# Naxaes/Rust-Swift-Raytracer

Measured on AMD Instinct MI355X. Metric: Mrays/sec + frames/sec at 1920×1080 spp=64; 1/2/4/8 MI355X, higher is better.
Workload: dtype f32; 1 GPU; c2: 1920x1080, spp 64, depth 8, 486 spheres, 0 triangles, COUNTER RNG; width=1920, height=1080, spp=64, depth=8, parallelism=one device renders the frame in place (no RCCL call)

## Files before the change

### rust-swift-raytracer_amd/csrc/render.h

```cpp
#pragma once

#include <hip/hip_runtime.h>

#include <cstdint>

#include "fastdiv.h"

namespace rtamd {

enum : uint32_t { kRngCounter = 1, kRngReplay = 2 };
enum : uint32_t { kRngSerialCount = 3, kRngSerialEstimate = 4, kRngSerialCheck = 5, kRngSerialCoalesce = 6,
                  kRngSerialPixel = 7 };
enum : uint32_t { kMatDiffuse = 0, kMatMetal = 1, kMatDielectric = 2, kMatEmission = 3 };
constexpr uint32_t kPrimaryTriStripW = 8;
#ifndef RT_TRACE_RING
#define RT_TRACE_RING 4
#endif
constexpr uint32_t kTraceRing = RT_TRACE_RING;
#ifdef RT_STAMPS
constexpr uint32_t kStatSlots = 24;
#else
constexpr uint32_t kStatSlots = 16;
#endif
constexpr uint32_t kStampSegs = 8;
// ... 16 lines not shown
    const float4 *tri_hot;
    const float4 *tri_geo;
    const float *mats;
    float *samples;
    float *ring;
    uint32_t ring_shift;
    uint32_t *out;
    float inv_spp;
    uint32_t alpha_u8;
    uint32_t *job_counter;
    uint32_t *job_counter_next;
    unsigned long long *stats;
    const uint32_t *replay;
    float cam[12];
    float wden, hden;
    float wrcp, hrcp;
    uint32_t xdiv_uv;
    uint32_t nsph, nsph_padded, ntri;
    uint32_t width, height, spp;
    int32_t depth;
    uint32_t mode, seed;
    uint32_t row_block, rank, nranks;
    uint32_t slab_row0;
    uint32_t njobs;
    uint32_t npix;
    uint32_t chunk;
    uint32_t nparts;
    const float4 *bvh_nodes;
    const uint32_t *bvh_miss;
    const uint16_t *bvh_miss16;
    const float4 *bvh_prims;
    const uint32_t *bvh_prim_id;
    const float4 *big_hot;
    const uint32_t *big_id;
    uint32_t nnodes, nbig, nprims;
    uint32_t use_lds;
    uint32_t ablate;
    const float4 *sph_shade;
    const uint32_t *sph_kind;
    FastDiv div_spp, div_width, div_rowblock;
    uint32_t refill_min;
    uint32_t walk_min;
    uint32_t tri_walk_min;
    uint32_t steps;
    uint32_t step;
    float bvh_c[3], bvh_r, bvh_rmax, bvh_mag, bvh_inv_rmin;
    const uint4 *tbvh_nodes;
    const float4 *tbvh_tris;
    const uint32_t *tbvh_loose;
    uint32_t tnodes, ttris, tloose;
    float tbvh_c[3], tbvh_r, tbvh_mag;
    float tbvh_oc[3];
    float tq_base[3], tq_step[3], tq_nbase, tq_nstep;
    const uint4 *tw_nodes;
    uint32_t tw_depth;
    uint32_t wsteps;
    float cq_base[3], cq_step[3];
    const uint4 *cam_nodes;
    const float4 *cam_tris;
    uint32_t cam_nnodes;
    const uint32_t *ptl_off;
    const uint32_t *ptl_items;
    uint32_t ptl_spr;
    uint32_t ptl_always, ptl_end;
    const uint2 *spl;
    const uint32_t *win;
    SerialPred sM;
    const uint32_t *slo;
    const uint32_t *ctrl;
    uint32_t cbase;
    uint32_t nserial;
    uint32_t sspp;
    FastDiv div_sspp;
    uint32_t max_draws;
    uint32_t sL, sK;
    uint32_t gj32, gj_c0, gj_2p;
    const float4 *tw_tris;
    uint32_t tw_stride, tc_ncells;
    uint32_t tc_n[3];
    float tc_lo[3], tc_size, tc_inv_size;
    const uint4 *spix;
};

RT_HOST_DEVICE inline uint32_t serial_lo(const SerialPred &M, uint32_t a, uint32_t jl, uint32_t K,
                                         uint32_t depth, uint32_t nserial) {
    const uint32_t j = a + jl < nserial ? a + jl : nserial;
    double c = __builtin_floor(serial_M(M, j) - serial_M(M, a)) - (double)(K / 2u);
    const double hi = (double)depth * (double)jl;
    c = c < 0.0 ? 0.0 : c;
    c = c > hi ? hi : c;
    return (uint32_t)c;
}

hipError_t launch_trace(const TraceParams &p, uint32_t blocks, hipStream_t stream,
                        const uint4 *corner = nullptr);
hipError_t launch_sphere_lists(const float4 *prims, uint32_t n, const double *Mi, const double *o,
                               double e_abs, double wden, double hden, uint32_t width, uint32_t height,
                               int4 *rects, uint32_t *flag, uint2 *rec, hipStream_t stream);
size_t serial_tab_doubles(uint32_t npix);
hipError_t launch_serial_check_count(const float *flags, uint32_t n, unsigned long long *count,
                                     hipStream_t stream);
hipError_t launch_serial_moments(const float *est, uint32_t pix0, uint32_t n, uint32_t spp, uint32_t R,
                                 double scale, double *tab, uint32_t npix, hipStream_t stream);
hipError_t launch_serial_tables(double *tab, double *scratch, uint32_t npix, uint32_t spp, uint32_t L,
                                uint32_t n0, hipStream_t stream);
size_t serial_scan_scratch(uint32_t npix);
constexpr uint32_t kSerialWinPerThread = 4;
constexpr uint32_t kSerialJumpT1 = 4096 / kSerialWinPerThread;
constexpr uint32_t kSerialJumpWords = 32 * (64 + kSerialJumpT1 + 256);
hipError_t launch_serial_window(uint32_t *ctrl, const uint32_t *jump, uint32_t *win, uint32_t n,
                                SerialPred M, uint32_t *lo, uint32_t L, uint32_t K, uint32_t depth,
                                uint32_t nserial, uint32_t pix_spp, uint32_t pix_emax, uint32_t *counters,
                                uint32_t ncounters, uint4 *spix, uint32_t pix_chunk, const uint4 *spix_prev,
                                hipStream_t stream);
hipError_t launch_serial_reuse(const uint32_t *ctrl, const uint4 *spix, const uint4 *spix_prev, float *ptab,
                               const float *ptab_prev, uint32_t npq_max, uint32_t spp, uint32_t L,
                               uint32_t nserial, hipStream_t stream);
hipError_t launch_serial_pixtab_gather(const uint32_t *ctrl, const float *ptab, const uint32_t *lo, float *table,
                                       uint32_t L, uint32_t K, uint32_t spp, uint32_t nserial, hipStream_t stream);
inline uint64_t serial_pixtab_emax64(uint64_t spp, uint64_t K, uint64_t depth) {
    return 2u * (spp - 1u) + 3u * (depth * (spp - 1u) + K) + 1u;
}
hipError_t launch_serial_coalesce(const TraceParams &p, uint32_t *path, uint32_t *bend, uint32_t L, uint32_t Kmax,
                                  uint32_t R, bool tree_lds, unsigned long long *dbg, hipStream_t stream);
size_t serial_coalesce_lds(const TraceParams &p, uint32_t K, bool tree_lds);
size_t serial_coalesce_search_lds(uint32_t K, uint32_t depth);
uint32_t serial_walk_block(uint32_t L);
constexpr uint32_t kMaxWalkBlocks = 4096;
constexpr uint32_t kWalkFinWords = 4 + kMaxWalkBlocks;
constexpr uint32_t kMaxWalkR = 256;
constexpr uint32_t kWalkLdsRowBytes = 48 * 1024;
constexpr uint32_t kWalkLdsMaxPix = 72;
hipError_t launch_serial_walk(uint32_t *ctrl, const float *table, SerialPred M, const double *V,
                              uint32_t npix, uint32_t spp, float z, float sfloor, const uint32_t *win,
                              uint32_t *states, uint32_t *bend, uint32_t *path, uint32_t *fin,
                              const uint32_t *lo, uint32_t *sbend, uint32_t *sB, uint32_t L, uint32_t Lw,
                              uint32_t K, uint32_t R, uint32_t depth, uint32_t nserial, const float *ptab,
                              uint32_t lds_rows, hipStream_t stream);
uint32_t serial_super_words(uint32_t L, uint32_t K, uint32_t R);
hipError_t launch_resolve_ex(const float *samples, uint32_t *out, uint32_t npix, uint32_t spp,
                             float inv_spp, uint32_t width, uint32_t slab_row0,
                             hipStream_t stream);
hipError_t launch_assemble(const uint32_t *gathered, uint32_t *out, uint32_t width, uint32_t height,
                           uint32_t row_block, uint32_t nranks, uint32_t max_rows,
                           hipStream_t stream);
hipError_t trace_occupancy(int *blocks_per_cu, int variant, size_t lds_bytes, bool step, int mesh,
                           int kind);
inline int trace_mesh_kind(bool triangles, bool tree) { return !triangles ? 0 : tree ? 2 : 1; }
size_t trace_lds_bytes(const TraceParams &p, bool corner = false);
__host__ __device__ inline size_t trace_tree_lds(uint32_t nnodes, uint32_t nprims, uint32_t nsph_padded) {
    return (size_t)nnodes * 64 + (size_t)nprims * 20 + (size_t)nsph_padded * 36;
}
__host__ __device__ inline size_t trace_corner_lds(uint32_t nnodes, uint32_t nprims) {
    return (size_t)nnodes * 128 + (size_t)nprims * 20;
}
constexpr size_t kLdsPerCu = 160 * 1024, kLdsDefaultMax = 64 * 1024;
hipError_t trace_lds_opt_in();
constexpr uint32_t kLdsTreeMaxNodes = 1023;
uint32_t trace_block_threads(bool lds, int mesh, int kind);
size_t trace_dyn_lds(const TraceParams &p, bool lds, bool wide, uint32_t threads, bool corner = false);

}
```

### rust-swift-raytracer_amd/csrc/render.hip

```cpp
#include <hip/hip_runtime.h>

#include <cstdint>
#include <type_traits>

#include "exactdiv.h"
#include "render.h"

#pragma clang fp contract(off)

namespace rtamd {
namespace {

struct F3 { float x, y, z; };

__device__ __forceinline__ F3 f3(float x, float y, float z) { return F3{x, y, z}; }
__device__ __forceinline__ F3 operator+(F3 a, F3 b) { return F3{a.x + b.x, a.y + b.y, a.z + b.z}; }
__device__ __forceinline__ F3 operator-(F3 a, F3 b) { return F3{a.x - b.x, a.y - b.y, a.z - b.z}; }
__device__ __forceinline__ F3 operator-(F3 a) { return F3{-a.x, -a.y, -a.z}; }
__device__ __forceinline__ F3 scale(F3 a, float s) { return F3{a.x * s, a.y * s, a.z * s}; }
__device__ __forceinline__ float dot(F3 a, F3 b) { return (a.x * b.x + a.y * b.y) + a.z * b.z; }
__device__ __forceinline__ F3 cross(F3 a, F3 b) {
    return F3{a.y * b.z - a.z * b.y, -(a.x * b.z - a.z * b.x), a.x * b.y - a.y * b.x};
}
__device__ __forceinline__ F3 divide_by(F3 a, float b) {
// ... 148 lines not shown
    const float r2 = -hb + sq;
    const bool v1 = tmin < r1;
    const float c = v1 ? r1 : r2;
    const bool valid = v1 || (tmin < r2);
    const uint64_t kc = ((uint64_t)__float_as_uint(c) << 32) | (uint32_t)idx;
    const uint64_t kb = ((uint64_t)__float_as_uint(best_t) << 32) | (uint32_t)best_i;
    const bool take = valid && c != __builtin_inff() && kc < kb;
    if (take) { best_t = c; best_i = idx; }
    return take;
}

constexpr float kErrK = 3.0e-3f;

struct BvhView {
    const float4 *nodes;
    const uint32_t *miss32;
    const uint16_t *miss16;
    const float4 *prims;
    const uint32_t *ids;
    const float4 *shade;
    const uint32_t *kinds;
};

__device__ __forceinline__ float slab_rcp(float d) {
    return __builtin_amdgcn_fmed3f(__builtin_amdgcn_rcpf(d), -1e20f, 1e20f);
}

struct SphBound { float A, e_abs; };
__device__ __forceinline__ SphBound sph_bound(const TraceParams &p, F3 org) {
    const float ax = org.x - p.bvh_c[0], ay = org.y - p.bvh_c[1], az = org.z - p.bvh_c[2];
    return SphBound{__builtin_amdgcn_sqrtf((ax * ax + ay * ay) + az * az) * 1.00001f + p.bvh_r,
                    2e-6f * ((fabsf(org.x) + fabsf(org.y)) + fabsf(org.z) + p.bvh_mag)};
}
constexpr float kErrKq = 40.5f * 0x1p-24f;
__device__ __forceinline__ float sph_inflation(const TraceParams &p, SphBound b, float bt) {
    const float s = fminf(b.A, bt + p.bvh_rmax) * (1.0f + 3.0f * kErrK) + p.bvh_rmax;
    return fminf(kErrK * s, (kErrKq * s) * (s * p.bvh_inv_rmin)) + b.e_abs;
}

__device__ __forceinline__ void spheres_big(const TraceParams &p, F3 org, F3 dir, float &best_t,
                                            int &best_i) {
    for (uint32_t k = 0; k < p.nbig; ++k) {
        const float4 S = uniform_load(p.big_hot, k);
        sphere_candidate(S, org, dir, (int)uniform_load_u32(p.big_id, k), best_t, best_i);
    }
}

template <bool kLds>
__device__ __forceinline__ bool sphere_node(const BvhView &v, F3 inv, uint32_t ooff, float best_t, F3 nlo,
                                            F3 nhi, uint32_t &node, uint32_t &leaf, uint32_t &node_tests) {
    ++node_tests;
    float4 B0, B1;
    uint32_t miss, hit = 0;
    if (kLds) {
#if defined(__HIP_DEVICE_COMPILE__)
        typedef const __attribute__((address_space(3))) char *lds_cptr;
        const lds_cptr rec = (lds_cptr)(uintptr_t)node;
        B0 = *(const __attribute__((address_space(3))) float4 *)rec;
        B1 = *(const __attribute__((address_space(3))) float4 *)(rec + 16);
        const uint32_t lw = *(const __attribute__((address_space(3))) uint32_t *)(rec + 32 + ooff);
        hit = lw & 0xFFFFu;
        miss = lw >> 16;
#else
        B0 = B1 = make_float4(0.0f, 0.0f, 0.0f, 0.0f);
        miss = 0;
#endif
    } else {
        B0 = v.nodes[2 * node];
        B1 = v.nodes[2 * node + 1];
        miss = v.miss32[8 * node + ooff];
    }
    const float t0x = __builtin_fmaf(B0.x, inv.x, nlo.x), t1x = __builtin_fmaf(B1.x, inv.x, nhi.x);
    const float t0y = __builtin_fmaf(B0.y, inv.y, nlo.y), t1y = __builtin_fmaf(B1.y, inv.y, nhi.y);
    const float t0z = __builtin_fmaf(B0.z, inv.z, nlo.z), t1z = __builtin_fmaf(B1.z, inv.z, nhi.z);
    const float tn = fmaxf(fmaxf(fminf(t0x, t1x), fminf(t0y, t1y)), fminf(t0z, t1z));
    const float tf = fminf(fminf(fmaxf(t0x, t1x), fmaxf(t0y, t1y)), fmaxf(t0z, t1z));
    const bool skip = tn > tf || tf < 0.001f || __float_as_int(tn) > __float_as_int(best_t);
    if (kLds) {
        leaf = __float_as_uint(B0.w);
        node = skip ? miss : hit;
        return !skip && leaf != 0u;
    }
    const uint32_t a = __float_as_uint(B0.w);
    const bool is_leaf = (a & kLeafBitDev) != 0;
    const uint32_t child = a + ((ooff >> __float_as_uint(B1.w)) & 1u);
    node = (skip || is_leaf) ? miss : child;
    leaf = ((a & ~kLeafBitDev) << 3) | __float_as_uint(B1.w);
    return !skip && is_leaf;
}

__device__ __forceinline__ bool sphere_node_corner(uint32_t offn, uint32_t offf, F3 inv, float best_t, F3 nn,
                                                   F3 nf, uint32_t &node, uint32_t &leaf, uint32_t &node_tests) {
    ++node_tests;
#if defined(__HIP_DEVICE_COMPILE__)
    typedef float f3v __attribute__((ext_vector_type(3)));
    uint32_t an, af;
    asm("v_lshl_add_u32 %0, %1, 7, %2" : "=v"(an) : "v"(node), "v"(offn));
    asm("v_lshl_add_u32 %0, %1, 7, %2" : "=v"(af) : "v"(node), "v"(offf));
    const float4 N = *(const __attribute__((address_space(3))) float4 *)(uintptr_t)an;
    const f3v Fc = *(const __attribute__((address_space(3))) f3v *)(uintptr_t)af;
    const float tnx = __builtin_fmaf(N.x, inv.x, nn.x), tfx = __builtin_fmaf(Fc.x, inv.x, nf.x);
    const float tny = __builtin_fmaf(N.y, inv.y, nn.y), tfy = __builtin_fmaf(Fc.y, inv.y, nf.y);
    const float tnz = __builtin_fmaf(N.z, inv.z, nn.z), tfz = __builtin_fmaf(Fc.z, inv.z, nf.z);
    const float tn = fmaxf(fmaxf(tnx, tny), tnz);
    const float tf = fminf(fminf(tfx, tfy), tfz);
    const bool skip = tn > tf || tf < 0.001f || __float_as_int(tn) > __float_as_int(best_t);
    const uint32_t lw = __float_as_uint(N.w);
    const bool is_leaf = (int32_t)lw < 0;
    node = (skip || is_leaf) ? (lw & 0xFFFFu) : (lw >> 16);
    leaf = (lw >> 16) & 0x7FFFu;
    return !skip && is_leaf;
#else
    (void)offn; (void)offf; (void)inv; (void)best_t; (void)nn; (void)nf;
    node = 0xFFFFu;
    leaf = 0;
    return false;
#endif
}

__device__ __forceinline__ uint32_t sphere_corner_entry(uint32_t lbase, uint32_t oct, uint32_t nnodes) {
#if defined(__HIP_DEVICE_COMPILE__)
    if (nnodes > 1u)
        return *(const __attribute__((address_space(3))) uint32_t *)(uintptr_t)(lbase + 16u * oct + 12u) >> 16;
#endif
    (void)lbase; (void)oct; (void)nnodes;
    return 0;
}

__device__ __forceinline__ void sphere_corner_slabs(F3 org, F3 inv, float e, uint32_t oct, F3 &nn, F3 &nf) {
    const float ex = (oct & 1u) ? -e : e, ey = (oct & 2u) ? -e : e, ez = (oct & 4u) ? -e : e;
    nn = f3(-((org.x + ex) * inv.x), -((org.y + ey) * inv.y), -((org.z + ez) * inv.z));
    nf = f3(-((org.x - ex) * inv.x), -((org.y - ey) * inv.y), -((org.z - ez) * inv.z));
}

template <bool kLds>
__device__ __forceinline__ uint32_t sphere_walk_entry(uint32_t root, uint32_t oct, uint32_t nnodes) {
#if defined(__HIP_DEVICE_COMPILE__)
    if (kLds && nnodes > 1u) {
        typedef const __attribute__((address_space(3))) char *lds_cptr;
        return *(const __attribute__((address_space(3))) uint32_t *)((lds_cptr)(uintptr_t)root + 32 + 4u * oct) &
               0xFFFFu;
    }
#endif
    (void)oct;
    (void)nnodes;
    return root;
}

__device__ __forceinline__ void sphere_slabs(F3 org, F3 inv, float e, F3 &nlo, F3 &nhi) {
    nlo = f3(-((org.x + e) * inv.x), -((org.y + e) * inv.y), -((org.z + e) * inv.z));
    nhi = f3(-((org.x - e) * inv.x), -((org.y - e) * inv.y), -((org.z - e) * inv.z));
}

__device__ __forceinline__ void sphere_leaf(const BvhView &v, F3 org, F3 dir, uint32_t leaf, float &best_t,
                                            int &best_i, uint32_t &sph_tests) {
    const uint32_t first = leaf >> 3, n = leaf & 7u;
#ifndef RT_LEAF_LOOP
    sph_tests += n;
    sphere_candidate(v.prims[first], org, dir, (int)v.ids[first], best_t, best_i);
    if (n > 1u) {
        sphere_candidate(v.prims[first + 1], org, dir, (int)v.ids[first + 1], best_t, best_i);
        for (uint32_t j = first + 2; j < first + n; ++j)
            sphere_candidate(v.prims[j], org, dir, (int)v.ids[j], best_t, best_i);
    }
#else
    for (uint32_t j = first; j < first + n; ++j) {
        ++sph_tests;
        sphere_candidate(v.prims[j], org, dir, (int)v.ids[j], best_t, best_i);
    }
#endif
}

__device__ __forceinline__ bool tri_edges(F3 n, F3 v0, F3 v1, F3 v2, F3 pt) {
    if (dot(n, cross(v1 - v0, pt - v0)) < 0.0f) return false;
    if (dot(n, cross(v2 - v1, pt - v1)) < 0.0f) return false;
    if (dot(n, cross(v0 - v2, pt - v2)) < 0.0f) return false;
    return true;
}

__device__ __forceinline__ bool tri_plane(float4 N, F3 org, F3 dir, float best_t, float &t) {
    const float cosl = (N.x * dir.x + N.y * dir.y) + N.z * dir.z;
    if (-1e-8f < cosl && cosl < 1e-8f) return false;
    t = (((N.x * org.x + N.y * org.y) + N.z * org.z) + N.w) / cosl;
    return !(t < 0.001f || t > best_t);
}

__device__ __forceinline__ void triangles_brute(const TraceParams &p, F3 org, F3 dir, float best_t,
                                                float &tri_t, int &tri_i, uint32_t &tri_in) {
    const float tmin = 0.001f;
    for (uint32_t j = 0; j < p.ntri; ++j) {
        const float4 N = p.tri_hot[j];
        const float cosl = (N.x * dir.x + N.y * dir.y) + N.z * dir.z;
        if (-1e-8f < cosl && cosl < 1e-8f) continue;
        const float t = (((N.x * org.x + N.y * org.y) + N.z * org.z) + N.w) / cosl;
        if (t < tmin || t > best_t) continue;
        ++tri_in;
        const float4 *g = p.tri_geo + 4u * j;
        const float4 A = g[0], B = g[1], Cc = g[2];
        if (!tri_edges(f3(N.x, N.y, N.z), f3(A.x, A.y, A.z), f3(B.x, B.y, B.z), f3(Cc.x, Cc.y, Cc.z),
                       org + scale(dir, t)))
            continue;
        if (t < tri_t) { tri_t = t; tri_i = (int)j; }
    }
}

__device__ __forceinline__ bool tri_merge(float t, int idx, float &tri_t, int &tri_i) {
    const bool take = t < tri_t || (t == tri_t && tri_t < __builtin_inff() && idx < tri_i);
    if (take) { tri_t = t; tri_i = idx; }
    return take;
}

__device__ __forceinline__ bool tri_record(const float4 *r, F3 org, F3 dir, float best_t,
                                           float &tri_t, int &tri_i, uint32_t &tri_in) {
    const float4 N = r[0];
    float t;
    if (!tri_plane(N, org, dir, best_t, t)) return false;
    ++tri_in;
    const float4 A = r[1], B = r[2], Cc = r[3];
    if (!tri_edges(f3(N.x, N.y, N.z), f3(A.x, A.y, A.z), f3(B.x, B.y, B.z), f3(Cc.x, Cc.y, Cc.z),
                   org + scale(dir, t)))
        return false;
    return tri_merge(t, (int)__float_as_uint(A.w), tri_t, tri_i);
}

__device__ __forceinline__ bool tri_begin(const TraceParams &p, F3 org, F3 dir, float best_t,
                                          bool cam, float &rho, float &tri_t, int &tri_i,
                                          uint32_t &tri_in, uint32_t &tri_done) {
    tri_done += p.tloose;
    for (uint32_t k = 0; k < p.tloose; ++k) {
        const uint32_t j = p.tbvh_loose[k];
        const float4 N = p.tri_hot[j];
        float t;
        if (!tri_plane(N, org, dir, best_t, t)) continue;
        ++tri_in;
        const float4 *g = p.tri_geo + 4u * j;
        const float4 A = g[0], B = g[1], Cc = g[2];
        if (tri_edges(f3(N.x, N.y, N.z), f3(A.x, A.y, A.z), f3(B.x, B.y, B.z), f3(Cc.x, Cc.y, Cc.z),
                      org + scale(dir, t)))
            tri_merge(t, (int)j, tri_t, tri_i);
    }
    const float onorm = (fabsf(org.x) + fabsf(org.y)) + fabsf(org.z);
    if (!cam && !(onorm < 1e18f)) {
        tri_done += p.ttris;
        for (uint32_t j = 0; j < p.ttris; ++j)
            tri_record(p.tbvh_tris + 4u * j, org, dir, best_t, tri_t, tri_i, tri_in);
        return false;
    }
    const float dist = ((fabsf(org.x - p.tbvh_c[0]) + fabsf(org.y - p.tbvh_c[1])) +
                        fabsf(org.z - p.tbvh_c[2])) + p.tbvh_r + 2.0f * onorm;
    rho = cam ? 0.0f : 1e-5f * ((dist + onorm) + p.tbvh_mag);
    return true;
}

__device__ __forceinline__ bool tri_node(const TraceParams &p, F3 nlo, F3 nhi, F3 inv, F3 dlt2, bool cam,
                                         float cap, uint32_t &node, uint32_t &leaf,
                                         uint32_t &node_tests) {
    ++node_tests;
    const uint4 *qn = (cam ? p.cam_nodes : p.tbvh_nodes) + 2u * node;
    const uint4 q0 = qn[0], q1 = qn[1];
    const uint32_t a = cam ? q0.w : q1.z;
    const uint32_t miss = cam ? q1.x : q1.w;
    const float gbx = cam ? p.cq_base[0] : p.tq_base[0], gsx = cam ? p.cq_step[0] : p.tq_step[0];
    const float gby = cam ? p.cq_base[1] : p.tq_base[1], gsy = cam ? p.cq_step[1] : p.tq_step[1];
    const float gbz = cam ? p.cq_base[2] : p.tq_base[2], gsz = cam ? p.cq_step[2] : p.tq_step[2];
    auto lo16 = [](uint32_t w) { return (float)(w & 0xFFFFu); };
    auto hi16 = [](uint32_t w) { return (float)(w >> 16); };
    const float4 B0 = make_float4(__builtin_fmaf(lo16(q0.x), gsx, gbx), __builtin_fmaf(hi16(q0.x), gsy, gby),
                                  __builtin_fmaf(lo16(q0.y), gsz, gbz), 0.0f);
    const float4 B1 = make_float4(__builtin_fmaf(hi16(q0.y), gsx, gbx), __builtin_fmaf(lo16(q0.z), gsy, gby),
                                  __builtin_fmaf(hi16(q0.z), gsz, gbz), 0.0f);
    const float nb = cam ? 0.0f : p.tq_nbase, ns = cam ? 0.0f : p.tq_nstep;
    const float4 N0 = make_float4(__builtin_fmaf(lo16(q0.w), ns, nb), __builtin_fmaf(hi16(q0.w), ns, nb),
                                  __builtin_fmaf(lo16(q1.x), ns, nb), 0.0f);
    const float4 N1 = make_float4(__builtin_fmaf(hi16(q1.x), ns, nb), __builtin_fmaf(lo16(q1.y), ns, nb),
                                  __builtin_fmaf(hi16(q1.y), ns, nb), 0.0f);
    const float ax = N0.x * dlt2.x, bx = N1.x * dlt2.x;
    const float ay = N0.y * dlt2.y, by = N1.y * dlt2.y;
    const float az = N0.z * dlt2.z, bz = N1.z * dlt2.z;
    const float sl = (fminf(ax, bx) + fminf(ay, by)) + fminf(az, bz);
    const float sh = (fmaxf(ax, bx) + fmaxf(ay, by)) + fmaxf(az, bz);
    auto widen = [&](float lo, float hi, float m0, float m1, float nl, float nh, float iv, float &t0,
                     float &t1) {
        const float a = sl * m0, b = sl * m1, c = sh * m0, d = sh * m1;
        const float omin = fminf(fminf(a, b), fminf(c, d));
        const float omax = fmaxf(fmaxf(a, b), fmaxf(c, d));
        t0 = __builtin_fmaf(lo + omin, iv, nl);
        t1 = __builtin_fmaf(hi + omax, iv, nh);
    };
    float t0x, t1x, t0y, t1y, t0z, t1z;
    widen(B0.x, B1.x, N0.x, N1.x, nlo.x, nhi.x, inv.x, t0x, t1x);
    widen(B0.y, B1.y, N0.y, N1.y, nlo.y, nhi.y, inv.y, t0y, t1y);
    widen(B0.z, B1.z, N0.z, N1.z, nlo.z, nhi.z, inv.z, t0z, t1z);
    const float tn = fmaxf(fmaxf(fminf(t0x, t1x), fminf(t0y, t1y)), fminf(t0z, t1z));
    const float tf = fminf(fminf(fmaxf(t0x, t1x), fmaxf(t0y, t1y)), fmaxf(t0z, t1z));
    const bool skip = tn > tf || tf < 0.001f || __float_as_int(tn) > __float_as_int(cap);
    const bool is_leaf = (a & kLeafBitDev) != 0;
    const uint32_t child = a & 0x1FFFFFFFu;
    node = (skip || is_leaf) ? miss : child;
    leaf = a & ~kLeafBitDev;
    return !skip && is_leaf;
}

__device__ __forceinline__ bool tri_wide_child(const TraceParams &p, uint32_t w0, uint32_t w1, uint32_t w2,
                                               uint32_t w3, uint32_t w4, uint32_t w5, F3 nlo, F3 nhi,
                                               F3 inv, F3 dlt2, float cap, float &tn) {
    auto lo16 = [](uint32_t w) { return (float)(w & 0xFFFFu); };
    auto hi16 = [](uint32_t w) { return (float)(w >> 16); };
    const float gsx = p.tq_step[0], gsy = p.tq_step[1], gsz = p.tq_step[2];
    auto h16lo = [](uint32_t w) { return (float)__builtin_bit_cast(_Float16, (uint16_t)(w & 0xFFFFu)); };
    auto h16hi = [](uint32_t w) { return (float)__builtin_bit_cast(_Float16, (uint16_t)(w >> 16)); };
    const float nx0 = h16lo(w3), ny0 = h16hi(w3), nz0 = h16lo(w4);
    const float nx1 = h16hi(w4), ny1 = h16lo(w5), nz1 = h16hi(w5);
    const float ax = nx0 * dlt2.x, bx = nx1 * dlt2.x;
    const float ay = ny0 * dlt2.y, by = ny1 * dlt2.y;
    const float az = nz0 * dlt2.z, bz = nz1 * dlt2.z;
    const float sl = (fminf(ax, bx) + fminf(ay, by)) + fminf(az, bz);
    const float sh = (fmaxf(ax, bx) + fmaxf(ay, by)) + fmaxf(az, bz);
    auto widen = [&](float qlo, float qhi, float m0, float m1, float c0, float c1, float gs, float iv, float &t0,
                     float &t1) {
        const float a = sl * m0, b = sl * m1, c = sh * m0, d = sh * m1;
        const float omin = fminf(fminf(a, b), fminf(c, d));
        const float omax = fmaxf(fmaxf(a, b), fmaxf(c, d));
        t0 = __builtin_fmaf(__builtin_fmaf(qlo, gs, omin), iv, c0);
        t1 = __builtin_fmaf(__builtin_fmaf(qhi, gs, omax), iv, c1);
    };
    float t0x, t1x, t0y, t1y, t0z, t1z;
    widen(lo16(w0), hi16(w1), nx0, nx1, nlo.x, nhi.x, gsx, inv.x, t0x, t1x);
    widen(hi16(w0), lo16(w2), ny0, ny1, nlo.y, nhi.y, gsy, inv.y, t0y, t1y);
    widen(lo16(w1), hi16(w2), nz0, nz1, nlo.z, nhi.z, gsz, inv.z, t0z, t1z);
    tn = fmaxf(fmaxf(fminf(t0x, t1x), fminf(t0y, t1y)), fminf(t0z, t1z));
    const float tf = fminf(fminf(fmaxf(t0x, t1x), fmaxf(t0y, t1y)), fmaxf(t0z, t1z));
    return !(tn > tf || tf < 0.001f || __float_as_int(tn) > __float_as_int(cap));
}

__device__ __forceinline__ void tri_leaf(const TraceParams &p, F3 org, F3 dir, bool cam,
                                         uint32_t leaf, float best_t, float &tri_t, int &tri_i,
                                         uint32_t &tri_in, uint32_t &tri_done, const float4 *wrecs = nullptr) {
    const float4 *recs = wrecs ? wrecs : cam ? p.cam_tris : p.tbvh_tris;
    const uint32_t first = leaf >> 3, end = first + (leaf & 7u);
    tri_done += leaf & 7u;
    for (uint32_t j = first; j < end; ++j)
        tri_record(recs + 4u * j, org, dir, best_t, tri_t, tri_i, tri_in);
}

template <bool kSerial>
__device__ __forceinline__ void job_pixel(const TraceParams &p, uint32_t job, uint32_t &s,
                                          uint32_t &col, uint32_t &row) {
    if (kSerial && p.mode == kRngSerialPixel) {
        const uint32_t pix = fdiv(p.cbase, p.div_sspp) + fdiv(job, p.div_spp);
        s = 0;
        row = fdiv(pix, p.div_width);
        col = pix - row * p.width;
        return;
    }
    if (kSerial) {
        const uint32_t jl = fdiv(job, p.div_spp);
        const uint32_t j = p.cbase + jl < p.nserial ? p.cbase + jl : p.nserial - 1u;
        const uint32_t pix = fdiv(j, p.div_sspp);
        s = j - pix * p.sspp;
        row = fdiv(pix, p.div_width);
        col = pix - row * p.width;
        return;
    }
    const uint32_t lp = fdiv(job, p.div_spp);
    s = job - lp * p.spp;
    const uint32_t q = fdiv(lp, p.div_width);
    col = lp - q * p.width;
    const uint32_t lr = p.slab_row0 + q;
    const uint32_t blk = fdiv(lr, p.div_rowblock);
    const uint32_t ir = (blk * p.nranks + p.rank) * p.row_block + (lr - blk * p.row_block);
    row = p.height - 1u - ir;
}

__device__ __forceinline__ void serial_pixel_span(const TraceParams &p, uint32_t q, uint32_t &plo,
                                                  uint32_t &phi) {
    if (p.spix != nullptr) {
        const uint4 s = p.spix[q];
        plo = s.x;
        phi = s.y;
        return;
    }
    const uint32_t a = p.cbase, ss = p.sspp;
    const uint32_t ln = min(p.sL, p.nserial - a);
    const uint32_t p0 = fdiv(a, p.div_sspp);
    const uint32_t jf = q == 0u ? 0u : (p0 + q) * ss - a;
    const uint32_t jz = min((p0 + q + 1u) * ss - a, ln) - 1u;
    plo = 2u * jf + 3u * p.slo[jf];
    phi = 2u * jz + 3u * (p.slo[jz] + p.sK - 1u);
}

__device__ __forceinline__ uint32_t serial_start(const TraceParams &p, uint32_t job) {
    const uint32_t jl = fdiv(job, p.div_spp);
    const uint32_t k = job - jl * p.spp;
    if (p.mode == kRngSerialCount)
        return p.win[2u * jl + 3u * ((p.slo ? p.slo[jl]
                                            : serial_lo(p.sM, p.cbase, jl, p.spp, (p.max_draws - 2u) / 3u,
                                                        p.nserial)) + k)];
    if (p.mode == kRngSerialCheck) return p.win[p.cbase + jl];
    if (p.mode == kRngSerialPixel) {
        uint32_t plo, phi;
        serial_pixel_span(p, jl, plo, phi);
        return p.win[min(plo + k, max(phi, plo))];
    }
    return counter_seed(p.seed, (uint64_t)(p.cbase + jl) * p.spp + k);
}

__device__ __forceinline__ bool serial_pixel_job(const TraceParams &p, uint32_t job) {
    const uint32_t q = fdiv(job, p.div_spp);
    uint32_t plo, phi;
    serial_pixel_span(p, q, plo, phi);
    return plo + (job - q * p.spp) <= phi;
}

template <bool kSerial>
__device__ __forceinline__ void tri_primary_list(const TraceParams &p, uint32_t job, F3 org, F3 dir,
                                                 float best_t, float &tri_t, int &tri_i,
                                                 uint32_t &tri_in, uint32_t &tri_done) {
    uint32_t s, col, row;
    job_pixel<kSerial>(p, job, s, col, row);
    const uint32_t strip = row * p.ptl_spr + col / kPrimaryTriStripW;
    const uint32_t b = p.ptl_off[strip], e = p.ptl_off[strip + 1];
    tri_done += (e - b) + (p.ptl_end - p.ptl_always);
    for (uint32_t j = b; j < e; ++j)
        tri_record(p.cam_tris + 4u * p.ptl_items[j], org, dir, best_t, tri_t, tri_i, tri_in);
    for (uint32_t j = p.ptl_always; j < p.ptl_end; ++j)
        tri_record(p.cam_tris + 4u * p.ptl_items[j], org, dir, best_t, tri_t, tri_i, tri_in);
}

__device__ __forceinline__ void resolve_store(const TraceParams &p, uint32_t lp, float r, float g,
                                              float b) {
    const uint32_t R = sat_u8(__builtin_sqrtf(r * p.inv_spp) * 255.999f);
    const uint32_t G = sat_u8(__builtin_sqrtf(g * p.inv_spp) * 255.999f);
    const uint32_t B = sat_u8(__builtin_sqrtf(b * p.inv_spp) * 255.999f);
    const uint32_t q = fdiv(lp, p.div_width);
    const uint32_t col = lp - q * p.width;
    p.out[(size_t)(p.slab_row0 + q) * p.width + col] = R | (G << 8) | (B << 16) | (p.alpha_u8 << 24);
}

#define RT_PLANE_LANES(mesh) ((mesh) < 2 || (mesh) == 3)
template <bool kPlaneLanes>
__device__ __forceinline__ void resolve_chunk(const TraceParams &p, const float *ring, uint32_t plane,
                                              uint32_t off, uint32_t base, uint32_t len,
                                              uint32_t lane) {
    __builtin_amdgcn_fence(__ATOMIC_RELEASE, "workgroup");
    __builtin_amdgcn_fence(__ATOMIC_ACQUIRE, "workgroup");
    const uint32_t spp = p.spp;
    const uint32_t np = fdiv(len, p.div_spp), pix0 = fdiv(base, p.div_spp);
    if (kPlaneLanes && 3u * np <= kWave && (spp & 3u) == 0) {
        const uint32_t c = lane >= np ? (lane >= 2u * np ? 2u : 1u) : 0u;
        const uint32_t g = lane - c * np;
        const bool on = lane < 3u * np;
        const float *src = ring + off + c * plane + (on ? g : 0u) * spp;
        float acc = 0.0f;
        for (uint32_t k = 0; k < spp; k += 16u) {
            float4 v[4];
#pragma unroll
            for (uint32_t q = 0; q < 4; ++q) {
                v[q] = make_float4(0.0f, 0.0f, 0.0f, 0.0f);
                if (on && k + 4u * q < spp) v[q] = *reinterpret_cast<const float4 *>(src + k + 4u * q);
            }
#pragma unroll
            for (uint32_t q = 0; q < 4; ++q) {
                if (k + 4u * q < spp) {
                    acc = acc + v[q].x;
                    acc = acc + v[q].y;
                    acc = acc + v[q].z;
                    acc = acc + v[q].w;
                }
            }
        }
        const float sg = __shfl(acc, (int)(lane < np ? np + lane : lane));
        const float sb = __shfl(acc, (int)(lane < np ? 2u * np + lane : lane));
        if (lane < np) resolve_store(p, pix0 + lane, acc, sg, sb);
        return;
    }
    for (uint32_t i = lane; i < np; i += kWave) {
        const float *src = ring + off + i * spp;
        float r = 0.0f, g = 0.0f, b = 0.0f;
        for (uint32_t k = 0; k < spp; ++k) {
            r = r + src[k];
            g = g + src[plane + k];
            b = b + src[2 * plane + k];
        }
        resolve_store(p, pix0 + i, r, g, b);
    }
}

template <bool kLds, bool kCorner>
__device__ __forceinline__ uint32_t stage_tree(const TraceParams &p, const uint4 *corner, float4 *lds,
                                               BvhView &view) {
    if (!kLds) {
        view = BvhView{p.bvh_nodes, p.bvh_miss, nullptr, p.bvh_prims, p.bvh_prim_id,
                       p.sph_shade, p.sph_kind};
        return 0;
    }
    float4 *n4 = lds;
    const uint32_t lbase = (uint32_t)(uintptr_t)(__attribute__((address_space(3))) float4 *)lds;
    if (kCorner) {
        float4 *c4 = n4 + 8u * p.nnodes;
        uint32_t *cid = reinterpret_cast<uint32_t *>(c4 + p.nprims);
        const float4 *g = reinterpret_cast<const float4 *>(corner);
        for (uint32_t i = threadIdx.x; i < 8u * p.nnodes; i += blockDim.x) n4[i] = g[i];
        for (uint32_t i = threadIdx.x; i < p.nprims; i += blockDim.x) {
            c4[i] = p.bvh_prims[i];
            cid[i] = p.bvh_prim_id[i];
        }
        __syncthreads();
        view = BvhView{n4, nullptr, nullptr, c4, cid, p.sph_shade, p.sph_kind};
        return lbase;
    }
    float4 *p4 = n4 + 4 * p.nnodes;
    float4 *s4 = p4 + p.nprims;
    uint32_t *id = reinterpret_cast<uint32_t *>(s4 + 2 * p.nsph_padded);
    uint32_t *kd = id + p.nprims;
    const uint16_t *g16 = p.bvh_miss16;
    auto addr = [&](uint32_t l) { return l == 0xFFFFu ? 0xFFFFu : lbase + l * 64u; };
    for (uint32_t i = threadIdx.x; i < p.nnodes; i += blockDim.x) {
        float4 b0 = p.bvh_nodes[2 * i];
        const uint32_t a = __float_as_uint(b0.w);
        float4 b1 = p.bvh_nodes[2 * i + 1];
        const bool is_leaf = (a & kLeafBitDev) != 0;
        const uint32_t axis = __float_as_uint(b1.w);
        b0.w = __uint_as_float(is_leaf ? ((a & ~kLeafBitDev) << 3) | axis : 0u);
        b1.w = 0.0f;
        n4[4 * i] = b0;
        n4[4 * i + 1] = b1;
        uint32_t w[8];
        for (uint32_t o = 0; o < 8; ++o) {
            const uint32_t miss = addr(g16[8 * i + o]);
            const uint32_t next = is_leaf ? miss : lbase + (a + ((o >> axis) & 1u)) * 64u;
            w[o] = next | (miss << 16);
        }
        n4[4 * i + 2] = make_float4(__uint_as_float(w[0]), __uint_as_float(w[1]), __uint_as_float(w[2]),
                                    __uint_as_float(w[3]));
        n4[4 * i + 3] = make_float4(__uint_as_float(w[4]), __uint_as_float(w[5]), __uint_as_float(w[6]),
                                    __uint_as_float(w[7]));
    }
    for (uint32_t i = threadIdx.x; i < p.nprims; i += blockDim.x) {
        p4[i] = p.bvh_prims[i];
        id[i] = p.bvh_prim_id[i];
    }
    for (uint32_t i = threadIdx.x; i < p.nsph_padded; i += blockDim.x) {
        s4[2 * i] = p.sph_shade[2 * i];
        s4[2 * i + 1] = p.sph_shade[2 * i + 1];
        kd[i] = p.sph_kind[i];
    }
    __syncthreads();
    view = BvhView{n4, nullptr, nullptr, p4, id, s4, kd};
    return lbase;
}

#ifndef RT_WAVES_PER_EU
#define RT_WAVES_PER_EU 6
#endif
#ifndef RT_WAVES_PER_EU_MESH
#define RT_WAVES_PER_EU_MESH 6
#endif
#ifndef RT_WAVES_PER_EU_SPHERES
#define RT_WAVES_PER_EU_SPHERES 8
#endif
#ifndef RT_LDS_BLOCK_SPHERES
#define RT_LDS_BLOCK_SPHERES 1024
#endif
#ifndef RT_WAVES_PER_EU_SPHERES_GLOBAL
#define RT_WAVES_PER_EU_SPHERES_GLOBAL 6
#endif
#ifndef RT_LDS_BLOCK_SPHERES_AUX
#define RT_LDS_BLOCK_SPHERES_AUX 768
#endif
#ifndef RT_LDS_BLOCK_MESH
#define RT_LDS_BLOCK_MESH 512
#endif
#ifndef RT_WAVES_PER_EU_WIDE
#define RT_WAVES_PER_EU_WIDE 6
#endif
#ifndef RT_LDS_BLOCK_WIDE
#define RT_LDS_BLOCK_WIDE 512
#endif
constexpr uint32_t trace_threads(bool lds, int mesh, int kind) {
    return !lds ? 256u : mesh == 3 ? (uint32_t)RT_LDS_BLOCK_WIDE : mesh ? (uint32_t)RT_LDS_BLOCK_MESH
                       : kind == 0 ? (uint32_t)RT_LDS_BLOCK_SPHERES : (uint32_t)RT_LDS_BLOCK_SPHERES_AUX;
}
constexpr int trace_waves_per_eu(bool lds, int mesh, int kind) {
    return kind != 0 ? RT_WAVES_PER_EU : mesh == 3 ? RT_WAVES_PER_EU_WIDE : mesh ? RT_WAVES_PER_EU_MESH
                       : lds ? RT_WAVES_PER_EU_SPHERES : RT_WAVES_PER_EU_SPHERES_GLOBAL;
}
template <bool kBvh, bool kLds, bool kStep, int kMesh, bool kCount, bool kSerial, bool kCorner>
__device__ __forceinline__ void trace_body(TraceParams p, const uint4 *corner) {
    if (kSerial && p.ctrl != nullptr) {
        if (p.ctrl[0] != 0u) return;
        p.cbase = p.ctrl[4];
        const uint32_t K = p.ctrl[5];
        if (p.mode == kRngSerialCount && K != 0u && K < p.spp) {
            if (p.chunk % p.spp == 0u) p.chunk = (p.chunk / K) * K;
            p.spp = K;
            p.div_spp = make_fastdiv(K);
            p.njobs = p.npix * K;
        }
        if (p.mode == kRngSerialPixel) {
            p.sK = K != 0u && K < p.sK ? K : p.sK;
            const uint32_t E = min(p.ctrl[7], p.spp);
            const uint32_t ln = min(p.sL, p.nserial - p.cbase);
            const uint32_t p0 = fdiv(p.cbase, p.div_sspp);
            const uint32_t npq = E ? fdiv(p.cbase + ln - 1u, p.div_sspp) - p0 + 1u : 0u;
            p.spp = max(E, 1u);
            p.div_spp = make_fastdiv(p.spp);
            p.npix = npq;
            p.njobs = npq * E;
        }
    }
    if (!kSerial && p.job_counter_next != nullptr && blockIdx.x == 0)
        for (uint32_t i = threadIdx.x; i < kMaxJobParts; i += blockDim.x) p.job_counter_next[32u * i] = 0u;
    const uint32_t lane = __lane_id();
    auto kargs = [&]() -> const TraceParams & {
#if defined(__HIP_DEVICE_COMPILE__) && !defined(RT_NO_KARG_RELOAD)
        if (kSerial) return p;
        const __attribute__((address_space(4))) TraceParams *kp =
            (const __attribute__((address_space(4))) TraceParams *)__builtin_amdgcn_kernarg_segment_ptr();
        asm volatile("" : "+s"(kp));
        return *(const TraceParams *)kp;
#else
        return p;
#endif
    };
    extern __shared__ float4 lds[];
    BvhView view;
    const uint32_t sph_root = stage_tree<kLds, kCorner>(p, corner, lds, view);
    uint16_t *const tstack = reinterpret_cast<uint16_t *>(
                                 reinterpret_cast<char *>(lds) +
                                 (kLds ? (trace_tree_lds(p.nnodes, p.nprims, p.nsph_padded) + 15u) & ~(size_t)15u
                                       : 0u)) + threadIdx.x;
    uint32_t tsp = 0;

    F3 org = f3(0, 0, 0), dir = f3(0, 0, 0), inv = f3(0, 0, 0);
    float thr_r = 1.0f, thr_g = 1.0f, thr_b = 1.0f;
    uint32_t rng = 0, slot = ~0u, bounce = 0;
    uint32_t nscat = 0;
    uint32_t spl0 = 0, spl1 = kSphListWalk << 16;
    enum : uint32_t { kSetup = 0, kSph = 1, kTriInit = 2, kTri = 3, kShade = 4 };
    uint32_t phase = kSetup, node = 0, oct = 0;
    float best_t = 0.0f, tri_t = 0.0f, e = 0.0f;
    int best_i = -1, tri_i = -1;
    bool active = false;
    uint32_t rays = 0, tri_in = 0, sph_tests = 0, node_tests = 0, tnode_tests = 0,
             tri_done = 0;
    uint32_t it_all = 0, it_walk = 0, lanes_all = 0, lanes_walk = 0;
#ifdef RT_WALK_MIX
    uint32_t wm_iters = 0, wm_leaf_iters = 0, wm_leaf_trips = 0, wm_walks = 0;
#endif

    uint32_t pool_next = 0, pool_end = 0;
    uint32_t gap_lo = ~0u, gap_len = 0;
    bool exhausted = false;

    const bool fused = p.ring != nullptr;
    const uint32_t wave_id = __builtin_amdgcn_readfirstlane(blockIdx.x * (blockDim.x / kWave) +
                                                            threadIdx.x / kWave);
    float *const sbase = fused ? p.ring + (size_t)wave_id * (3u * kTraceRing << p.ring_shift)
                               : p.samples;
    const uint32_t pstride = fused ? (kTraceRing << p.ring_shift) : p.njobs;
    uint32_t rfree = (1u << kTraceRing) - 1u;
    uint32_t rbase[kTraceRing], rlen[kTraceRing], rleft[kTraceRing];
#pragma unroll
    for (uint32_t k = 0; k < kTraceRing; ++k) rbase[k] = rlen[k] = rleft[k] = 0;
    uint32_t cur_off = 0;
    auto lane_job = [&](uint32_t sl) -> uint32_t {
        if (!fused) return sl;
        const uint32_t k = sl >> p.ring_shift;
        uint32_t b = rbase[0];
#pragma unroll
        for (uint32_t i = 1; i < kTraceRing; ++i) b = k == i ? rbase[i] : b;
        return b + (sl & ((1u << p.ring_shift) - 1u));
    };

#ifdef RT_WAVE_TIMES
    const uint64_t wt_start = __builtin_amdgcn_s_memrealtime();
    uint64_t wt_pull = wt_start, wt_exh = wt_start;
    uint32_t wt_jobs_tail = 0;
#endif
#ifdef RT_STAMPS
    uint64_t stamp_acc[kStampSegs] = {0, 0, 0, 0, 0, 0, 0, 0};
    uint64_t stamp_prev = __builtin_amdgcn_s_memtime();
#define RT_STAMP(k)                                                       \
    do {                                                                  \
        __builtin_amdgcn_sched_barrier(0);                                \
        const uint64_t t_ = __builtin_amdgcn_s_memtime();                 \
        __builtin_amdgcn_sched_barrier(0);                                \
        stamp_acc[k] += t_ - stamp_prev;                                  \
        stamp_prev = t_;                                                  \
    } while (0)
#else
#define RT_STAMP(k) \
    do {            \
    } while (0)
#endif
    uint32_t part = (blockIdx.x * (blockDim.x / kWave) + threadIdx.x / kWave) % p.nparts;
    uint32_t tries = 0;
    auto part_begin = [&](uint32_t k) -> uint32_t {
        return (uint32_t)(((uint64_t)k * p.npix) / p.nparts) * p.spp;
    };
    uint32_t pbegin = part_begin(part), pend = part_begin(part + 1);
    uint32_t prefetch = 0;
    bool prefetch_pending = false;
    for (;;) {
        F3 vdir = dir;
        bool renorm = false;
        bool done = false;
        bool walked = false;
        const uint32_t nact = kCount ? (uint32_t)__popcll(__ballot(active)) : 0u;
        if (active) {
            float out_r = 0.0f, out_g = 0.0f, out_b = 0.0f;
            if (phase == kSetup) {
                const TraceParams &p = kargs();
                if ((int32_t)bounce >= p.depth) {
                    done = true;
                } else {
                    ++rays;
                    inv = f3(slab_rcp(dir.x), slab_rcp(dir.y), slab_rcp(dir.z));
                    oct = (inv.x < 0.0f ? 1u : 0u) | (inv.y < 0.0f ? 2u : 0u) | (inv.z < 0.0f ? 4u : 0u);
                    best_t = __builtin_inff();
                    best_i = -1;
                    if (kBvh) {
                        spheres_big(p, org, dir, best_t, best_i);
                        node = kCorner ? sphere_corner_entry(sph_root, oct, p.nnodes)
                                                         : sphere_walk_entry<kLds>(sph_root, oct, p.nnodes);
                        phase = (p.ablate & 1u) ? kTriInit : kSph;
                        if (!kMesh && bounce == 0 && (spl1 >> 16) != kSphListWalk) {
                            const uint32_t nc = spl1 >> 16;
                            sph_tests += nc;
                            if (nc > 0) sphere_candidate(view.prims[spl0 & 0xFFFFu], org, dir,
                                                         (int)view.ids[spl0 & 0xFFFFu], best_t, best_i);
                            if (nc > 1) sphere_candidate(view.prims[spl0 >> 16], org, dir,
                                                         (int)view.ids[spl0 >> 16], best_t, best_i);
                            if (nc > 2) sphere_candidate(view.prims[spl1 & 0xFFFFu], org, dir,
                                                         (int)view.ids[spl1 & 0xFFFFu], best_t, best_i);
                            phase = kTriInit;
                        }
                    } else {
                        spheres_brute(p, org, dir, best_t, best_i);
                        phase = kTriInit;
                    }
                }
            }
            RT_STAMP(1);
            uint32_t budget = p.steps;
            bool walk_now = true;
            if (!kMesh && p.walk_min != 0) {
                const uint32_t nwalk = (uint32_t)__popcll(__ballot(phase == kSph));
                const uint32_t nother = (uint32_t)__popcll(__ballot(phase != kSph && !done));
                walk_now = nwalk >= p.walk_min || nother == 0;
            }
            if (kBvh && phase == kSph && walk_now) {
                const TraceParams &p = kargs();
                walked = true;
                constexpr uint32_t kEnd = kLds ? 0xFFFFu : kNodeEndDev;
                const SphBound bnd = sph_bound(p, org);
                if (kCorner) {
                    F3 nn, nf;
                    sphere_corner_slabs(org, inv, sph_inflation(p, bnd, best_t), oct, nn, nf);
                    const uint32_t offn = sph_root + 16u * oct, offf = sph_root + 112u - 16u * oct;
                    do {
                        uint32_t leaf;
                        if (sphere_node_corner(offn, offf, inv, best_t, nn, nf, node, leaf, node_tests))
                            sphere_leaf(view, org, dir, leaf, best_t, best_i, sph_tests);
                    } while (node != 0xFFFFu && (!kStep || --budget != 0));
                } else {
                    F3 nlo, nhi;
                    sphere_slabs(org, inv, sph_inflation(p, bnd, best_t), nlo, nhi);
                    const uint32_t ooff = kLds ? 4u * oct : oct;
#ifdef RT_WALK_MIX
                    uint32_t wi = 0, wl = 0, wt = 0;
#endif
                    do {
                        uint32_t leaf;
                        const bool lf = sphere_node<kLds>(view, inv, ooff, best_t, nlo, nhi, node, leaf, node_tests);
#ifdef RT_WALK_MIX
                        if (kCount) {
                            ++wi;
                            const bool any1 = __ballot(lf) != 0;
                            const bool any2 = __ballot(lf && (leaf & 7u) >= 2u) != 0;
                            wl += any1 ? 1u : 0u;
                            wt += any2 ? 2u : any1 ? 1u : 0u;
                        }
#endif
                        if (lf) sphere_leaf(view, org, dir, leaf, best_t, best_i, sph_tests);
                    } while (node != kEnd && (!kStep || --budget != 0));
#ifdef RT_WALK_MIX
                    if (kCount) {
                        for (uint32_t off = 1; off < kWave; off <<= 1) {
                            wi = max(wi, (uint32_t)__shfl_xor((int)wi, (int)off));
                            wl = max(wl, (uint32_t)__shfl_xor((int)wl, (int)off));
                            wt = max(wt, (uint32_t)__shfl_xor((int)wt, (int)off));
                        }
                        wm_iters += wi;
                        wm_leaf_iters += wl;
                        wm_leaf_trips += wt;
                        wm_walks += 1u;
                    }
#endif
                }
                if (node == kEnd) phase = kTriInit;
            }
            if (phase == kTriInit) {
                const TraceParams &p = kargs();
                tri_t = __builtin_inff();
                tri_i = -1;
                phase = kShade;
                if (kMesh == 0) {
                } else if (kMesh >= 2) {
                    const bool cam = kMesh == 2 && bounce == 0 && p.cam_nnodes != 0;
                    if (tri_begin(p, org, dir, best_t, cam, e, tri_t, tri_i, tri_in, tri_done)) {
                        if (bounce == 0 && p.ptl_off != nullptr) {
                            tri_primary_list<kSerial>(p, lane_job(slot), org, dir, best_t, tri_t, tri_i, tri_in,
                                             tri_done);
                        } else {
                            node = 0;
                            tsp = 0;
                            phase = kTri;
                        }
                    }
                } else {
                    triangles_brute(p, org, dir, best_t, tri_t, tri_i, tri_in);
                }
            }
            bool tri_now = true;
            if (kMesh >= 2 && p.tri_walk_min != 0) {
                const uint32_t nwalk = (uint32_t)__popcll(__ballot(phase == kTri));
                const uint32_t nother = (uint32_t)__popcll(__ballot(phase != kTri && !done));
                tri_now = nwalk >= p.tri_walk_min || nother == 0;
            }
            if (kMesh == 2 && phase == kTri && tri_now) {
                const TraceParams &p = kargs();
                if (kStep) budget = max(budget, p.steps / 2u);
                const bool cam = bounce == 0 && p.cam_nnodes != 0;
                const F3 dlt2 = f3(2.0f * (org.x - p.tbvh_oc[0]), 2.0f * (org.y - p.tbvh_oc[1]),
                                   2.0f * (org.z - p.tbvh_oc[2]));
                F3 nlo, nhi;
                sphere_slabs(org, inv, e, nlo, nhi);
                float cap = fminf(best_t, tri_t);
                do {
                    uint32_t leaf;
                    if (tri_node(p, nlo, nhi, inv, dlt2, cam, cap, node, leaf, tnode_tests)) {
                        tri_leaf(p, org, dir, cam, leaf, best_t, tri_t, tri_i, tri_in, tri_done);
                        cap = fminf(best_t, tri_t);
                    }
                } while (node != kNodeEndDev && (!kStep || --budget != 0));
                if (node == kNodeEndDev) phase = kShade;
            }
            if (kMesh == 3 && phase == kTri && tri_now) {
                const TraceParams &p = kargs();
                uint32_t wbudget = p.wsteps;
                F3 oc = f3(p.tbvh_oc[0], p.tbvh_oc[1], p.tbvh_oc[2]);
                uint32_t tree = 0;
                if (p.tc_ncells != 0u) {
                    const float fx = floorf((org.x - p.tc_lo[0]) * p.tc_inv_size);
                    const float fy = floorf((org.y - p.tc_lo[1]) * p.tc_inv_size);
                    const float fz = floorf((org.z - p.tc_lo[2]) * p.tc_inv_size);
                    tree = p.tc_ncells;
                    if (fx >= 0.0f && fx < (float)p.tc_n[0] && fy >= 0.0f && fy < (float)p.tc_n[1] && fz >= 0.0f &&
                        fz < (float)p.tc_n[2]) {
                        tree = ((uint32_t)fz * p.tc_n[1] + (uint32_t)fy) * p.tc_n[0] + (uint32_t)fx;
                        oc = f3(p.tc_lo[0] + (fx + 0.5f) * p.tc_size, p.tc_lo[1] + (fy + 0.5f) * p.tc_size,
                                p.tc_lo[2] + (fz + 0.5f) * p.tc_size);
                    }
                }
                const F3 dlt2 = f3(2.0f * (org.x - oc.x), 2.0f * (org.y - oc.y), 2.0f * (org.z - oc.z));
                F3 nlo, nhi;
                sphere_slabs(org, inv, e, nlo, nhi);
                nlo = f3(__builtin_fmaf(p.tq_base[0], inv.x, nlo.x), __builtin_fmaf(p.tq_base[1], inv.y, nlo.y),
                         __builtin_fmaf(p.tq_base[2], inv.z, nlo.z));
                nhi = f3(__builtin_fmaf(p.tq_base[0], inv.x, nhi.x), __builtin_fmaf(p.tq_base[1], inv.y, nhi.y),
                         __builtin_fmaf(p.tq_base[2], inv.z, nhi.z));
                float cap = fminf(best_t, tri_t);
                do {
                    const uint4 *wn = p.tw_nodes + 8u * (tree * p.tw_stride + node);
                    tnode_tests += 4;
                    float tn[4];
                    bool in[4];
#ifndef RT_WIDE_ONE_LOAD
                    {
                        const uint4 q0 = wn[0], q1 = wn[1], q2 = wn[2];
                        in[0] = tri_wide_child(p, q0.x, q0.y, q0.z, q0.w, q1.x, q1.y, nlo, nhi, inv, dlt2, cap, tn[0]);
                        in[1] = tri_wide_child(p, q1.z, q1.w, q2.x, q2.y, q2.z, q2.w, nlo, nhi, inv, dlt2, cap, tn[1]);
                    }
                    asm volatile("" ::: "memory");
                    {
                        const uint4 q3 = wn[3], q4 = wn[4], q5 = wn[5];
                        in[2] = tri_wide_child(p, q3.x, q3.y, q3.z, q3.w, q4.x, q4.y, nlo, nhi, inv, dlt2, cap, tn[2]);
                        in[3] = tri_wide_child(p, q4.z, q4.w, q5.x, q5.y, q5.z, q5.w, nlo, nhi, inv, dlt2, cap, tn[3]);
                    }
#else
                    {
                        const uint4 q0 = wn[0], q1 = wn[1], q2 = wn[2], q3 = wn[3], q4 = wn[4], q5 = wn[5];
                        in[0] = tri_wide_child(p, q0.x, q0.y, q0.z, q0.w, q1.x, q1.y, nlo, nhi, inv, dlt2, cap, tn[0]);
                        in[1] = tri_wide_child(p, q1.z, q1.w, q2.x, q2.y, q2.z, q2.w, nlo, nhi, inv, dlt2, cap, tn[1]);
                        in[2] = tri_wide_child(p, q3.x, q3.y, q3.z, q3.w, q4.x, q4.y, nlo, nhi, inv, dlt2, cap, tn[2]);
                        in[3] = tri_wide_child(p, q4.z, q4.w, q5.x, q5.y, q5.z, q5.w, nlo, nhi, inv, dlt2, cap, tn[3]);
                    }
#endif
                    const uint4 qa = wn[6];
                    const uint32_t a[4] = {qa.x, qa.y, qa.z, qa.w};
                    uint32_t lmask = 0;
#pragma unroll
                    for (int c = 0; c < 4; ++c) lmask |= (in[c] && (a[c] & kLeafBitDev)) ? 1u << c : 0u;
                    while (lmask != 0) {
                        const uint32_t c = (uint32_t)__builtin_ctz(lmask);
                        lmask &= lmask - 1u;
                        const uint32_t lw = c == 0 ? a[0] : c == 1 ? a[1] : c == 2 ? a[2] : a[3];
                        tri_leaf(p, org, dir, false, lw & ~kLeafBitDev, best_t, tri_t, tri_i, tri_in, tri_done,
                                 p.tw_tris);
                    }
                    cap = fminf(best_t, tri_t);
                    uint32_t nxt = 0xFFFFu;
                    float ntn = 0.0f;
#pragma unroll
                    for (int c = 3; c >= 0; --c) {
                        if (in[c] && !(a[c] & kLeafBitDev) && __float_as_int(tn[c]) <= __float_as_int(cap)) {
                            if (nxt != 0xFFFFu) {
                                const bool closer = tn[c] < ntn;
                                tstack[tsp * blockDim.x] = (uint16_t)(closer ? nxt : a[c]);
                                ++tsp;
                                if (closer) { nxt = a[c]; ntn = tn[c]; }
                            } else {
                                nxt = a[c];
                                ntn = tn[c];
                            }
                        }
                    }
                    if (nxt == 0xFFFFu && tsp != 0) {
                        --tsp;
                        nxt = tstack[tsp * blockDim.x];
                    }
                    node = nxt;
                } while (node != 0xFFFFu && (!kStep || --wbudget != 0));
                if (node == 0xFFFFu) phase = kShade;
            }
            RT_STAMP(2);
            if (phase == kShade) {
// ... 1725 lines not shown
```

Measured before the change: 64170 Mrays/s.

## Recompute walk state at BVH entry, prefetch second leaf sphere, shuffle packed channels

For sphere-only, non-stepped walks, the ray's reciprocal direction, octant and entry node are now computed at the start of the BVH walk instead of at ray setup. This shortens their live range and is meant to reduce register pressure across the phase machine. Leaf intersection can load the second sphere and its id before testing the first, to hide LDS/global latency; it reserves 16 extra LDS bytes so that read past the leaf stays in bounds. The resolve path now quantizes each channel to u8 before the cross-lane shuffle instead of shuffling floats and quantizing after, at the cost of one sqrt per lane.

```diff
diff --git a/rust-swift-raytracer_amd/csrc/render.h b/rust-swift-raytracer_amd/csrc/render.h
--- a/rust-swift-raytracer_amd/csrc/render.h
+++ b/rust-swift-raytracer_amd/csrc/render.h
@@ -192,7 +192,7 @@
     return (size_t)nnodes * 64 + (size_t)nprims * 20 + (size_t)nsph_padded * 36;
 }
 __host__ __device__ inline size_t trace_corner_lds(uint32_t nnodes, uint32_t nprims) {
-    return (size_t)nnodes * 128 + (size_t)nprims * 20;
+    return (size_t)nnodes * 128 + (size_t)nprims * 20 + 16;
 }
 constexpr size_t kLdsPerCu = 160 * 1024, kLdsDefaultMax = 64 * 1024;
 hipError_t trace_lds_opt_in();
diff --git a/rust-swift-raytracer_amd/csrc/render.hip b/rust-swift-raytracer_amd/csrc/render.hip
--- a/rust-swift-raytracer_amd/csrc/render.hip
+++ b/rust-swift-raytracer_amd/csrc/render.hip
@@ -324,14 +324,25 @@
     nhi = f3(-((org.x - e) * inv.x), -((org.y - e) * inv.y), -((org.z - e) * inv.z));
 }
 
+template <bool kAhead = false>
 __device__ __forceinline__ void sphere_leaf(const BvhView &v, F3 org, F3 dir, uint32_t leaf, float &best_t,
                                             int &best_i, uint32_t &sph_tests) {
     const uint32_t first = leaf >> 3, n = leaf & 7u;
 #ifndef RT_LEAF_LOOP
     sph_tests += n;
+    float4 S1 = make_float4(0.0f, 0.0f, 0.0f, 0.0f);
+    int i1 = 0;
+    if (kAhead) {
+        S1 = v.prims[first + 1];
+        i1 = (int)v.ids[first + 1];
+    }
     sphere_candidate(v.prims[first], org, dir, (int)v.ids[first], best_t, best_i);
     if (n > 1u) {
-        sphere_candidate(v.prims[first + 1], org, dir, (int)v.ids[first + 1], best_t, best_i);
+        if (!kAhead) {
+            S1 = v.prims[first + 1];
+            i1 = (int)v.ids[first + 1];
+        }
+        sphere_candidate(S1, org, dir, i1, best_t, best_i);
         for (uint32_t j = first + 2; j < first + n; ++j)
             sphere_candidate(v.prims[j], org, dir, (int)v.ids[j], best_t, best_i);
     }
@@ -599,14 +610,18 @@
         tri_record(p.cam_tris + 4u * p.ptl_items[j], org, dir, best_t, tri_t, tri_i, tri_in);
 }
 
-__device__ __forceinline__ void resolve_store(const TraceParams &p, uint32_t lp, float r, float g,
-                                              float b) {
-    const uint32_t R = sat_u8(__builtin_sqrtf(r * p.inv_spp) * 255.999f);
-    const uint32_t G = sat_u8(__builtin_sqrtf(g * p.inv_spp) * 255.999f);
-    const uint32_t B = sat_u8(__builtin_sqrtf(b * p.inv_spp) * 255.999f);
+__device__ __forceinline__ uint32_t resolve_channel(const TraceParams &p, float sum) {
+    return sat_u8(__builtin_sqrtf(sum * p.inv_spp) * 255.999f);
+}
+__device__ __forceinline__ void resolve_store_u8(const TraceParams &p, uint32_t lp, uint32_t R, uint32_t G,
+                                                 uint32_t B) {
     const uint32_t q = fdiv(lp, p.div_width);
     const uint32_t col = lp - q * p.width;
     p.out[(size_t)(p.slab_row0 + q) * p.width + col] = R | (G << 8) | (B << 16) | (p.alpha_u8 << 24);
+}
+__device__ __forceinline__ void resolve_store(const TraceParams &p, uint32_t lp, float r, float g,
+                                              float b) {
+    resolve_store_u8(p, lp, resolve_channel(p, r), resolve_channel(p, g), resolve_channel(p, b));
 }
 
 #define RT_PLANE_LANES(mesh) ((mesh) < 2 || (mesh) == 3)
@@ -641,9 +656,10 @@
                 }
             }
         }
-        const float sg = __shfl(acc, (int)(lane < np ? np + lane : lane));
-        const float sb = __shfl(acc, (int)(lane < np ? 2u * np + lane : lane));
-        if (lane < np) resolve_store(p, pix0 + lane, acc, sg, sb);
+        const uint32_t ch = resolve_channel(p, acc);
+        const uint32_t G = (uint32_t)__shfl((int)ch, (int)(lane < np ? np + lane : lane));
+        const uint32_t B = (uint32_t)__shfl((int)ch, (int)(lane < np ? 2u * np + lane : lane));
+        if (lane < np) resolve_store_u8(p, pix0 + lane, ch, G, B);
         return;
     }
     for (uint32_t i = lane; i < np; i += kWave) {
@@ -811,6 +827,7 @@
     uint32_t spl0 = 0, spl1 = kSphListWalk << 16;
     enum : uint32_t { kSetup = 0, kSph = 1, kTriInit = 2, kTri = 3, kShade = 4 };
     uint32_t phase = kSetup, node = 0, oct = 0;
+    constexpr bool kWalkState = kMesh == 0 && !kStep;
     float best_t = 0.0f, tri_t = 0.0f, e = 0.0f;
     int best_i = -1, tri_i = -1;
     bool active = false;
@@ -888,14 +905,17 @@
                     done = true;
                 } else {
                     ++rays;
-                    inv = f3(slab_rcp(dir.x), slab_rcp(dir.y), slab_rcp(dir.z));
-                    oct = (inv.x < 0.0f ? 1u : 0u) | (inv.y < 0.0f ? 2u : 0u) | (inv.z < 0.0f ? 4u : 0u);
+                    if (!kWalkState) {
+                        inv = f3(slab_rcp(dir.x), slab_rcp(dir.y), slab_rcp(dir.z));
+                        oct = (inv.x < 0.0f ? 1u : 0u) | (inv.y < 0.0f ? 2u : 0u) | (inv.z < 0.0f ? 4u : 0u);
+                    }
                     best_t = __builtin_inff();
                     best_i = -1;
                     if (kBvh) {
                         spheres_big(p, org, dir, best_t, best_i);
-                        node = kCorner ? sphere_corner_entry(sph_root, oct, p.nnodes)
-                                                         : sphere_walk_entry<kLds>(sph_root, oct, p.nnodes);
+                        if (!kWalkState)
+                            node = kCorner ? sphere_corner_entry(sph_root, oct, p.nnodes)
+                                           : sphere_walk_entry<kLds>(sph_root, oct, p.nnodes);
                         phase = (p.ablate & 1u) ? kTriInit : kSph;
                         if (!kMesh && bounce == 0 && (spl1 >> 16) != kSphListWalk) {
                             const uint32_t nc = spl1 >> 16;
@@ -927,6 +947,12 @@
                 walked = true;
                 constexpr uint32_t kEnd = kLds ? 0xFFFFu : kNodeEndDev;
                 const SphBound bnd = sph_bound(p, org);
+                if (kWalkState) {
+                    inv = f3(slab_rcp(dir.x), slab_rcp(dir.y), slab_rcp(dir.z));
+                    oct = (inv.x < 0.0f ? 1u : 0u) | (inv.y < 0.0f ? 2u : 0u) | (inv.z < 0.0f ? 4u : 0u);
+                    node = kCorner ? sphere_corner_entry(sph_root, oct, p.nnodes)
+                                   : sphere_walk_entry<kLds>(sph_root, oct, p.nnodes);
+                }
                 if (kCorner) {
                     F3 nn, nf;
                     sphere_corner_slabs(org, inv, sph_inflation(p, bnd, best_t), oct, nn, nf);
@@ -934,7 +960,7 @@
                     do {
                         uint32_t leaf;
                         if (sphere_node_corner(offn, offf, inv, best_t, nn, nf, node, leaf, node_tests))
-                            sphere_leaf(view, org, dir, leaf, best_t, best_i, sph_tests);
+                            sphere_leaf<true>(view, org, dir, leaf, best_t, best_i, sph_tests);
                     } while (node != 0xFFFFu && (!kStep || --budget != 0));
                 } else {
                     F3 nlo, nhi;
@@ -955,7 +981,7 @@
                             wt += any2 ? 2u : any1 ? 1u : 0u;
                         }
 #endif
-                        if (lf) sphere_leaf(view, org, dir, leaf, best_t, best_i, sph_tests);
+                        if (lf) sphere_leaf<kLds>(view, org, dir, leaf, best_t, best_i, sph_tests);
                     } while (node != kEnd && (!kStep || --budget != 0));
 #ifdef RT_WALK_MIX
                     if (kCount) {
```

Measured after the change: 65590 Mrays/s (median of 6 runs). +2.2%, better.
